# sjz5202/DisenLink

Measured on NVIDIA B200. Metric: factor-agg edges/s (fwd+bwd), higher is better.
Workload: dtype f32

## Files before the change

### disenlink_b200/csrc/attn_sym.cu

```cuda
#include "dl_dispatch.cuh"
#include "dl_prims.cuh"
#include "dl_stream.cuh"

namespace {

inline int blocks_for(long long n, int threads = 256) {
  long long b = (n + threads - 1) / threads;
  if (b < 1) b = 1;
  if (b > 148 * 32) b = 148 * 32;
  return (int)b;
}

__device__ __forceinline__ bool dl_primary(const long long* __restrict__ rowptr, int i, int j) {
  if (i == j) return true;
  const long long di = __ldg(rowptr + i + 1) - __ldg(rowptr + i), dj = __ldg(rowptr + j + 1) - __ldg(rowptr + j);
  return di > dj || (di == dj && i < j);
}

struct PrimaryFlag {
  const long long* rowptr;
  const int* col;
  const int* erow;
  long long nnz;
  __device__ __forceinline__ int operator()(long long e) const {
    return (e < nnz && dl_primary(rowptr, erow[e], col[e])) ? 1 : 0;
  }
};

__global__ void k_sym_uptr(const long long* __restrict__ rowptr, const int* __restrict__ pos, long long N,
                           long long* __restrict__ uptr) {
  const long long stride = (long long)gridDim.x * blockDim.x;
  for (long long r = (long long)blockIdx.x * blockDim.x + threadIdx.x; r <= N; r += stride) uptr[r] = pos[rowptr[r]];
}

__global__ void k_sym_fill(const long long* __restrict__ rowptr, const int* __restrict__ col,
                           const int* __restrict__ erow, long long nnz, const int* __restrict__ pos,
                           int* __restrict__ ucol, int* __restrict__ eidx,
                           int* __restrict__ lcol, int* __restrict__ lmirror, int* __restrict__ status,
                           unsigned long long* __restrict__ n_diag) {
  const long long stride = (long long)gridDim.x * blockDim.x;
  for (long long e = (long long)blockIdx.x * blockDim.x + threadIdx.x; e < nnz; e += stride) {
    const int i = erow[e], j = col[e];
    if (j == i) atomicAdd(n_diag, 1ULL);
    const int t = pos[e];
    if (pos[e + 1] != t) {
      ucol[t] = j;
      eidx[e] = t;
    } else {
      long long a = rowptr[j], b = rowptr[j + 1];
      const long long b0 = b;
      while (a < b) {
        const long long mid = (a + b) >> 1;
        if (col[mid] < i) a = mid + 1; else b = mid;
      }
      int m = 0;
      if (a < b0 && col[a] == i && pos[a + 1] != pos[a]) {
        m = pos[a];
      } else {
        *status = DL_EASYM;
      }
      eidx[e] = ~m;
      if (lcol) {
        lcol[e - t] = j;
        lmirror[e - t] = m;
      }
    }
  }
}

__global__ void k_sym_check(long long nnz, const int* __restrict__ pos,
                            const unsigned long long* __restrict__ n_diag, int* __restrict__ status) {
  const long long nu = pos[nnz];
  if (nnz - nu != nu - (long long)*n_diag) *status = DL_EASYM;
}

constexpr int SX_WARPS = 8;

template <int KP>
__global__ void __launch_bounds__(SX_WARPS * 32)
k_sym_expand(DlGraphDev g, const int* __restrict__ eidx, const float2* __restrict__ kw, int K,
             unsigned char* __restrict__ kstar, float* __restrict__ w, float* __restrict__ s,
             float* __restrict__ carry) {
  const int lane = threadIdx.x & 31;
  const long long gw = (long long)blockIdx.x * SX_WARPS + (threadIdx.x >> 5);
  const long long RE = (long long)DL_CH * DL_RANGE;
  DlChunkStream cs;
  cs.init(g.nnz, (long long)gridDim.x * SX_WARPS, g.range_shift);

  constexpr int NG = 32 / KP;
  const int grp = lane / KP, kap = lane % KP;
  float acc = 0.0f;
  int cur_row = -1;
  bool first_run = true, head_open = false, tail_open = false;
  long long cur_range = -1;
  auto flush = [&](bool at_range_end) {
    if (cur_row >= 0) {
      float v = acc;
#pragma unroll
      for (int off = KP; off < 32; off <<= 1) v = __fadd_rn(v, __shfl_xor_sync(DL_FULL, v, off));
      const bool to_head = first_run && head_open;
      const bool to_tail = !to_head && at_range_end && tail_open;
      if (grp == 0 && kap < K) {
        if (to_head || to_tail) carry[(cur_range * 2 + (to_tail ? 1 : 0)) * K + kap] = v;
        else s[(g.row_base + cur_row) * K + kap] = (v == 0.0f) ? 1.0f : v;
      }
      first_run = false;
    }
    cur_row = -1;
    acc = 0.0f;
  };

  struct Meta { int row, idx; };
  auto load_meta = [&](long long cc, Meta& m) {
    m.row = -1; m.idx = 0;
    if (cc >= 0) {
      const long long e = cc * DL_CH + lane;
      if (e < g.nnz) {
        m.row = __ldg(g.erow + e);
        const int t = __ldg(eidx + e);
        m.idx = t < 0 ? ~t : t;
      }
    }
  };
  auto gather = [&](const Meta& m) {
    float2 v = make_float2(0.0f, 0.0f);
    if (m.row >= 0) {
      asm volatile("ld.global.nc.L2::64B.v2.f32 {%0,%1}, [%2];" : "=f"(v.x), "=f"(v.y) : "l"(kw + m.idx));
    }
    return v;
  };

  long long c = cs.first(gw);
  Meta mA, mB, mC;
  load_meta(c, mA);
  long long cn = cs.next(c);
  load_meta(cn, mB);
  float2 vA = gather(mA), vB;
  while (c >= 0) {
    const long long cnn = cs.next(cn);
    load_meta(cnn, mC);
    vB = gather(mB);
    const long long rg = c >> g.range_shift;
    if (rg != cur_range) {
      if (cur_range >= 0) flush(true);
      cur_range = rg;
      first_run = true;
      const long long R0 = rg * RE, R1 = min(R0 + RE, g.nnz);
      head_open = R0 > 0 && __ldg(g.erow + R0 - 1) == __ldg(g.erow + R0);
      tail_open = R1 < g.nnz && __ldg(g.erow + R1) == __ldg(g.erow + R1 - 1);
    }
    const int ks = __float_as_int(vA.y);
    if (mA.row >= 0) {
      const long long e = c * DL_CH + lane;
      kstar[e] = (unsigned char)ks;
      w[e] = vA.x;
    }
    const unsigned vmask = __ballot_sync(DL_FULL, mA.row >= 0);
    const int cnt = __popc(vmask);
    for (int q = 0; q < cnt; q += NG) {
      const int src = q + grp;
      const int row_e = __shfl_sync(DL_FULL, mA.row, src & 31);
      const int ks_e = __shfl_sync(DL_FULL, ks, src & 31);
      const float w_e = __shfl_sync(DL_FULL, vA.x, src & 31);
      const bool valid = src < cnt;
      const float contrib = (valid && kap == ks_e) ? w_e : 0.0f;
      if (!__any_sync(DL_FULL, valid && row_e != cur_row)) {
        acc = __fadd_rn(acc, contrib);
      } else {
#pragma unroll 1
        for (int t = 0; t < NG && q + t < cnt; ++t) {
          const int re = __shfl_sync(DL_FULL, mA.row, q + t);
          if (re != cur_row) { flush(false); cur_row = re; }
          if (grp == t) acc = __fadd_rn(acc, contrib);
        }
      }
    }
    c = cn; cn = cnn;
    mA = mB; mB = mC;
    vA = vB;
  }
  if (cur_range >= 0) flush(true);
}

}

extern "C" {

size_t dl_sym_index_workspace_bytes(int64_t N, int64_t nnz) {
  if (N < 0 || nnz < 0) return 0;
  return dlp::align256((size_t)(nnz + 2) * 4) + dlp::scan_ws_bytes(nnz + 1, 4) + 256;
}

int dl_sym_index(const int64_t* rowptr, const int32_t* col, const int32_t* erow, int64_t N, int64_t nnz,
                 int64_t* uptr, int32_t* ucol, int32_t* eidx, int32_t* lcol, int32_t* lmirror, int32_t* status_out,
                 void* ws, size_t ws_bytes, dl_stream_t stream) {
  if (N < 0 || nnz < 0 || !rowptr || !uptr || !ws || (nnz > 0 && (!col || !erow))) return DL_EINVAL;
  if (ws_bytes < dl_sym_index_workspace_bytes(N, nnz)) return DL_EWORKSPACE;
  if (nnz >= 0x7fffffffLL) return DL_EUNSUPPORTED;
  cudaStream_t st = (cudaStream_t)stream;
  int* pos = (int*)ws;
  void* scan_ws = (char*)ws + dlp::align256((size_t)(nnz + 2) * 4);
  int rc = dlp::scan<false, int>(PrimaryFlag{(const long long*)rowptr, col, erow, nnz}, dlp::StoreArr<int>{pos}, nnz + 1,
                                 dlp::OpSum<int>(), 0, scan_ws, st);
  if (rc) return rc;
  if (!ucol) {
    k_sym_uptr<<<blocks_for(N + 1), 256, 0, st>>>((const long long*)rowptr, pos, N, (long long*)uptr);
    DL_LAUNCH_CHECK();
    return DL_OK;
  }
  if (!eidx || !status_out || ((lcol == nullptr) != (lmirror == nullptr))) return DL_EINVAL;
  DL_CUDA_TRY(cudaMemsetAsync(status_out, 0, sizeof(int32_t), st));
  unsigned long long* n_diag =
      (unsigned long long*)((char*)ws + dlp::align256((size_t)(nnz + 2) * 4) + dlp::scan_ws_bytes(nnz + 1, 4));
  DL_CUDA_TRY(cudaMemsetAsync(n_diag, 0, sizeof(unsigned long long), st));
  if (nnz > 0) {
    k_sym_fill<<<blocks_for(nnz), 256, 0, st>>>((const long long*)rowptr, col, erow, nnz, pos, ucol, eidx, lcol,
                                                lmirror, status_out, n_diag);
    DL_LAUNCH_CHECK();
    k_sym_check<<<1, 1, 0, st>>>(nnz, pos, n_diag, status_out);
    DL_LAUNCH_CHECK();
  }
  return DL_OK;
}

int dl_edge_attn_fwd_sym(const dl_graph* g_host, const dl_graph* upper_host, const int32_t* eidx, const float* Z,
                         int K, int d, float T, uint8_t* kstar, float* w, float* s, float* hub_ws, float* kw_scratch,
                         float* a_out, dl_stream_t stream) {
  if (!dl_graph_ok(g_host) || !dl_graph_ok(upper_host) || !dl_shape_ok(K, d)) return DL_EINVAL;
  if (g_host->N == 0) return DL_OK;
  if (g_host->row_base != 0 || upper_host->row_base != 0 || upper_host->N != g_host->N) return DL_EINVAL;
  if (!Z || !s || (g_host->nnz > 0 && (!kstar || !w || !eidx || !kw_scratch || !hub_ws))) return DL_EINVAL;
  if (!g_host->erow || !upper_host->erow) return DL_EINVAL;
  if (!(T == T) || T == 0.0f) return DL_EINVAL;
  if (!dl_attn_fl_has(K, d) || g_host->nnz == 0) return DL_EUNSUPPORTED;
  cudaStream_t st = (cudaStream_t)stream;
  const DlGraphDev g = dl_graph_dev(g_host);
  const DlGraphDev gu = dl_graph_dev(upper_host);
  float2* kw = reinterpret_cast<float2*>(kw_scratch);
  if (g_host->flags & DL_F_NO_KEEPA) a_out = nullptr;
  int rc = dl_launch_attn_fl(gu, Z, K, d, T, nullptr, nullptr, nullptr, nullptr, st, kw, a_out);
  if (rc == -1000) return DL_EUNSUPPORTED;
  if (rc) return rc;
  int dev = 0, sms = 0;
  DL_CUDA_TRY(cudaGetDevice(&dev));
  DL_CUDA_TRY(cudaDeviceGetAttribute(&sms, cudaDevAttrMultiProcessorCount, dev));
  const long long n_chunks = (g.nnz + DL_CH - 1) / DL_CH;
  const long long n_ranges = (n_chunks + DL_RANGE - 1) / DL_RANGE;
  long long grid = (n_ranges + SX_WARPS - 1) / SX_WARPS;
  if (grid > (long long)sms * 8) grid = (long long)sms * 8;
  if (grid < 1) grid = 1;
  if (K <= 8) k_sym_expand<8><<<(int)grid, SX_WARPS * 32, 0, st>>>(g, eidx, kw, K, kstar, w, s, hub_ws);
  else k_sym_expand<32><<<(int)grid, SX_WARPS * 32, 0, st>>>(g, eidx, kw, K, kstar, w, s, hub_ws);
  DL_LAUNCH_CHECK();
  return dl_gather_chain_rowsum(g, K, hub_ws, s, st);
}

}
```

### disenlink_b200/csrc/factor_fwd.cu

```cuda
#include <math_constants.h>
#include <stdlib.h>

#include "dl_dispatch.cuh"

namespace {

template <class M>
__global__ void __launch_bounds__(DL_CTA_S)
k_edge_attn_fwd(DlGraphDev g, const float* __restrict__ Z, float T, unsigned char* __restrict__ kstar,
                float* __restrict__ w, float* __restrict__ s, float* __restrict__ hub_ws) {
  constexpr int K = M::K, D = M::D, NP = M::NP, EB = M::EB, LP = M::LP, FPP = M::FPP;
  const int lane = threadIdx.x & 31;
  const long long warp0 = (long long)blockIdx.x * DL_WARPS_PER_CTA_S + (threadIdx.x >> 5);
  const long long nwarps = (long long)gridDim.x * DL_WARPS_PER_CTA_S;

  int off[NP];
  bool act[NP];
#pragma unroll
  for (int p = 0; p < NP; ++p) { off[p] = M::offset(lane, p); act[p] = M::active(lane, p); }
  const int my_e = M::edge_of_lane(lane);
  const int gsrc = lane & (EB - 1);
  const bool primary = (lane % LP) < EB;
  const bool unit_T = (T == 1.0f);

  auto fetch = [&](float4 (&dst)[EB][NP], int colreg, int idx0, int lim) {
#pragma unroll
    for (int e = 0; e < EB; ++e) {
      const int idx = idx0 + e;
      const int c = __shfl_sync(DL_FULL, colreg, idx & 31);
      const bool valid = idx < lim;
#pragma unroll
      for (int p = 0; p < NP; ++p)
        dst[e][p] = (valid && act[p]) ? dl_ldg4(Z + (long long)c * D + off[p]) : dl_zero4();
    }
  };

  DlRowIter itr;
  itr.init(g, warp0, nwarps);
  DlItem it, nit;
  it = nit = DlItem{0, 0, 0, 0, -1};
  bool have = itr.next(g, it);
  int colA = 0;
  if (have && lane < it.e1 - it.e0) colA = __ldg(g.col + it.e0 + lane);
  float4 zjA[EB][NP], zjB[EB][NP];
  bool pre = false;

  while (have) {
    const bool have_n = itr.next(g, nit);
    const int ncntB = have_n ? (int)min(32LL, nit.e1 - nit.e0) : 0;
    int colB = 0;
    if (lane < ncntB) colB = __ldg(g.col + nit.e0 + lane);
    float4 zi[NP];
#pragma unroll
    for (int p = 0; p < NP; ++p) zi[p] = act[p] ? dl_ldg4(Z + it.node * D + off[p]) : dl_zero4();
    if (!pre && it.e1 > it.e0) fetch(zjA, colA, 0, (int)min(32LL, it.e1 - it.e0));
    bool pre_n = false;

    float sacc[NP];
#pragma unroll
    for (int p = 0; p < NP; ++p) sacc[p] = 0.0f;
    int mycol = colA, colN = 0;
    for (long long base = it.e0; base < it.e1; base += 32) {
      const int cnt = (int)min(32LL, it.e1 - base);
      const bool more = base + 32 < it.e1;
      const int ncntN = more ? (int)min(32LL, it.e1 - base - 32) : 0;
      if (lane < ncntN) colN = __ldg(g.col + base + 32 + lane);
      int out_ks = 0;
      float out_w = 0.0f;
      const int nsub = (cnt + EB - 1) / EB;
      for (int sb = 0; sb < nsub; ++sb) {
        {
          int pc, pi0, plim;
          if (sb + 1 < nsub) { pc = mycol; pi0 = (sb + 1) * EB; plim = cnt; }
          else if (more) { pc = colN; pi0 = 0; plim = ncntN; }
          else { pc = colB; pi0 = 0; plim = ncntB; pre_n = ncntB > 0; }
          fetch(zjB, pc, pi0, plim);
        }
        float ev[NP];
#pragma unroll
        for (int p = 0; p < NP; ++p) {
          float part[EB];
#pragma unroll
          for (int e = 0; e < EB; ++e) part[e] = dl_chunk_dot(zi[p], zjA[e][p]);
          float q = dl_reduce_scatter<M>(part, lane);
          if (!unit_T) q = __fdiv_rn(q, T);
          ev[p] = dl_expf(q);
        }
        float a[K];
        float sum = 0.0f;
#pragma unroll
        for (int k = 0; k < K; ++k) {
          a[k] = __shfl_sync(DL_FULL, ev[k / FPP], (k % FPP) * LP + gsrc);
          sum = (k == 0) ? a[0] : __fadd_rn(sum, a[k]);
        }
        int ks = 0;
        float emax = a[0];
#pragma unroll
        for (int k = 1; k < K; ++k)
          if (a[k] > emax) { emax = a[k]; ks = k; }
        const float thr = __fmul_rn(emax, 0.99999976158142089844f);
        bool slow = !(sum < CUDART_INF_F);
#pragma unroll
        for (int k = 0; k < K; ++k) slow = slow || (a[k] > thr && a[k] != emax);
        float wv;
        if (!slow) {
          wv = __fdiv_rn(emax, sum);
        } else {
          ks = 0;
          wv = 0.0f;
#pragma unroll
          for (int k = 0; k < K; ++k) {
            float v = __fdiv_rn(a[k], sum);
            if (k == 0) { wv = v; }
            else if (v > wv || (v != v && wv == wv)) { wv = v; ks = k; }
          }
        }
        const bool valid = (sb * EB + my_e) < cnt;
#pragma unroll
        for (int p = 0; p < NP; ++p)
          if (valid && primary && ks == M::factor(lane, p)) sacc[p] = __fadd_rn(sacc[p], wv);
        if (sb == lane / EB) { out_ks = ks; out_w = wv; }
#pragma unroll
        for (int e = 0; e < EB; ++e)
#pragma unroll
          for (int p = 0; p < NP; ++p) zjA[e][p] = zjB[e][p];
      }
      const int oi = (lane & ~(EB - 1)) + my_e;
      if (oi < cnt) {
        kstar[base + oi] = (unsigned char)out_ks;
        w[base + oi] = out_w;
      }
      mycol = colN;
    }
#pragma unroll
    for (int p = 0; p < NP; ++p) {
      float v = sacc[p];
#pragma unroll
      for (int o = 1; o < EB; o <<= 1) v = __fadd_rn(v, __shfl_xor_sync(DL_FULL, v, o));
      const int k = M::factor(lane, p);
      if (k < K && (lane % LP) == 0) {
        if (it.hub_slot >= 0) hub_ws[it.hub_slot * K + k] = v;
        else s[it.node * K + k] = (v == 0.0f) ? 1.0f : v;
      }
    }
    it = nit;
    have = have_n;
    colA = colB;
    pre = pre_n;
  }
}

__global__ void __launch_bounds__(DL_CTA)
k_edge_attn_fwd_generic(DlGraphDev g, const float* __restrict__ Z, int K, int d, float T,
                        unsigned char* __restrict__ kstar, float* __restrict__ w,
                        float* __restrict__ s, float* __restrict__ hub_ws) {
  const int lane = threadIdx.x & 31;
  const long long warp0 = (long long)blockIdx.x * DL_WARPS_PER_CTA + (threadIdx.x >> 5);
  const long long nwarps = (long long)gridDim.x * DL_WARPS_PER_CTA;
  const long long n_items = dl_num_items(g);
  const long long D = (long long)K * d;
  float e[DL_MAX_K], a[DL_MAX_K], sacc[DL_MAX_K];
  for (long long t = warp0; t < n_items; t += nwarps) {
    const DlItem it = dl_decode_item(g, t);
    for (int k = 0; k < K; ++k) sacc[k] = 0.0f;
    const float* zi = Z + it.node * D;
    for (long long p = it.e0; p < it.e1; ++p) {
      const float* zj = Z + (long long)__ldg(g.col + p) * D;
      int ks = dl_generic_route(zi, zj, K, d, T, lane, e, a);
      float wv = a[ks];
      sacc[ks] = __fadd_rn(sacc[ks], wv);
      if (lane == 0) { kstar[p] = (unsigned char)ks; w[p] = wv; }
    }
    if (lane == 0) {
      for (int k = 0; k < K; ++k) {
        if (it.hub_slot >= 0) hub_ws[it.hub_slot * K + k] = sacc[k];
        else s[it.node * K + k] = (sacc[k] == 0.0f) ? 1.0f : sacc[k];
      }
    }
  }
}

__global__ void k_attn_hub_fixup(DlGraphDev g, int K, const float* __restrict__ hub_ws,
                                 float* __restrict__ s) {
  long long stride = (long long)gridDim.x * blockDim.x;
  for (long long x = (long long)blockIdx.x * blockDim.x + threadIdx.x; x < g.n_hub * K; x += stride) {
    long long h = x / K;
    int k = (int)(x % K);
    long long a = g.hub_seg_ptr[h], b = g.hub_seg_ptr[h + 1];
    float v = 0.0f;
    for (long long sg = a; sg < b; ++sg) v = __fadd_rn(v, hub_ws[sg * K + k]);
    s[(g.row_base + g.perm[h]) * K + k] = (v == 0.0f) ? 1.0f : v;
  }
}

__global__ void __launch_bounds__(DL_CTA)
k_factor_spmm_fwd_generic(DlGraphDev g, const float* __restrict__ Z,
                          const unsigned char* __restrict__ kstar, const float* __restrict__ w,
                          const float* __restrict__ s, int K, int d, float beta, float omb,
                          float* __restrict__ H, float* __restrict__ hub_ws) {
  const int lane = threadIdx.x & 31;
  const long long warp0 = (long long)blockIdx.x * DL_WARPS_PER_CTA + (threadIdx.x >> 5);
  const long long nwarps = (long long)gridDim.x * DL_WARPS_PER_CTA;
  const long long n_items = dl_num_items(g);
  const long long D = (long long)K * d;
  for (long long t = warp0; t < n_items; t += nwarps) {
    const DlItem it = dl_decode_item(g, t);
    float* acc = it.hub_slot >= 0 ? hub_ws + it.hub_slot * D : H + it.node * D;
    for (long long x = lane; x < D; x += 32) acc[x] = 0.0f;
    __syncwarp();
    for (long long p = it.e0; p < it.e1; ++p) {
      const long long j = __ldg(g.col + p);
      const int k = __ldg(kstar + p);
      const float coef = __fdiv_rn(__ldg(w + p), __ldg(s + j * K + k));
      const float* zj = Z + j * D + (long long)k * d;
      float* ak = acc + (long long)k * d;
      for (int x = lane; x < d; x += 32) ak[x] = __fmaf_rn(coef, zj[x], ak[x]);
    }
    __syncwarp();
    if (it.hub_slot < 0) {
      const float* zi = Z + it.node * D;
      for (long long x = lane; x < D; x += 32)
        acc[x] = __fadd_rn(__fmul_rn(beta, zi[x]), __fmul_rn(omb, acc[x]));
    }
  }
}

__global__ void k_spmm_hub_fixup(DlGraphDev g, long long D, const float* __restrict__ Z,
                                 const float* __restrict__ hub_ws, float beta, float omb,
                                 float* __restrict__ H) {
  long long stride = (long long)gridDim.x * blockDim.x;
  for (long long x = (long long)blockIdx.x * blockDim.x + threadIdx.x; x < g.n_hub * D; x += stride) {
    long long h = x / D, o = x % D;
    long long a = g.hub_seg_ptr[h], b = g.hub_seg_ptr[h + 1];
    float v = 0.0f;
    for (long long sg = a; sg < b; ++sg) v = __fadd_rn(v, hub_ws[sg * D + o]);
    long long row = g.row_base + g.perm[h];
    H[row * D + o] = __fadd_rn(__fmul_rn(beta, Z[row * D + o]), __fmul_rn(omb, v));
  }
}

template <class M>
int launch_attn(const DlGraphDev& g, long long n_items, const float* Z, float T, uint8_t* kstar,
                float* w, float* s, float* hub_ws, cudaStream_t st) {
  int grid = 1;
  int rc = dl_grid_for(k_edge_attn_fwd<M>, n_items, &grid, 0, DL_CTA_S);
  if (rc) return rc;
  k_edge_attn_fwd<M><<<grid, DL_CTA_S, 0, st>>>(g, Z, T, kstar, w, s, hub_ws);
  DL_LAUNCH_CHECK();
  return DL_OK;
}

inline int fixup_blocks(long long n) {
  long long b = (n + 255) / 256;
  if (b < 1) b = 1;
  if (b > 148 * 16) b = 148 * 16;
  return (int)b;
}

}

static __global__ void __launch_bounds__(256)
k_scale_rows(const float* __restrict__ Z, const float* __restrict__ s, long long n_rows, int K, int d,
             float* __restrict__ Zs) {
  const int lane = threadIdx.x & 31;
  const int D4 = K * d / 4, d4 = d / 4;
  const long long nwarps = (long long)gridDim.x * (blockDim.x >> 5);
  for (long long row = (long long)blockIdx.x * (blockDim.x >> 5) + (threadIdx.x >> 5); row < n_rows; row += nwarps) {
    const float4* zr = reinterpret_cast<const float4*>(Z) + row * D4;
    float4* out = reinterpret_cast<float4*>(Zs) + row * D4;
    for (int c = lane; c < D4; c += 32) {
      const float rs = __fdiv_rn(1.0f, __ldg(s + row * K + c / d4));
      float4 v = __ldg(zr + c);
      v.x = __fmul_rn(v.x, rs); v.y = __fmul_rn(v.y, rs); v.z = __fmul_rn(v.z, rs); v.w = __fmul_rn(v.w, rs);
      out[c] = v;
    }
  }
}

static __global__ void k_entry_sj(DlGraphDev g, const unsigned char* __restrict__ kstar, const float* __restrict__ s,
                           int K, float* __restrict__ sj) {
  const long long stride = (long long)gridDim.x * blockDim.x;
  for (long long e = (long long)blockIdx.x * blockDim.x + threadIdx.x; e < g.nnz; e += stride)
    sj[e] = __ldg(s + (long long)__ldg(g.col + e) * K + __ldg(kstar + e));
}

extern "C" {

size_t dl_hub_scratch_floats(const dl_graph* g_host, int64_t width) {
  if (!g_host || width < 0) return 0;
  const size_t hub = (size_t)g_host->n_hub_items * (size_t)width;
  const long long RE = 32LL << dl_range_shift(g_host->nnz);
  const size_t stream = (size_t)((g_host->nnz + RE - 1) / RE) * 3 * (size_t)width;
  return hub > stream ? hub : stream;
}

static int attn_fwd_impl(const dl_graph* g_host, const float* Z, int K, int d, float T,
                         uint8_t* kstar, float* w, float* s, float* hub_ws, float* const* s_peers, int n_peers,
                         dl_stream_t stream) {
  if (!dl_graph_ok(g_host) || !dl_shape_ok(K, d)) return DL_EINVAL;
  if (g_host->N == 0) return DL_OK;
  if (!Z || !s || (g_host->nnz > 0 && (!kstar || !w))) return DL_EINVAL;
  if (g_host->n_hub_items > 0 && !hub_ws) return DL_EINVAL;
  if (!(T == T) || T == 0.0f) return DL_EINVAL;
  cudaStream_t st = (cudaStream_t)stream;
  const unsigned flags = g_host->flags;
  const bool no_stream = (flags & DL_F_NO_STREAM) != 0;
  DlGraphDev g = dl_graph_dev(g_host);
  if (!dl_set_peer_out(g, s_peers, n_peers)) return DL_EINVAL;
  const long long n_items = g.n_hub_items + (g.N - g.n_hub);
  int rc = -1000;
  bool stream_tried = false;
  if (g.erow && g.nnz > 0 && !(flags & (DL_F_NO_STREAM | DL_F_NO_FL | DL_F_NO_FL_ATTN))) {
    rc = dl_launch_attn_fl(g, Z, K, d, T, kstar, w, s, hub_ws, st);
    if (rc == DL_OK) return DL_OK;
    if (rc != -1000) return rc;
  }
  if (g.erow && g.nnz > 0 && !no_stream) {
    rc = dl_launch_attn_stream(g, g.erow, Z, K, d, T, kstar, w, s, hub_ws, st);
    stream_tried = (rc != -1000);
  }
  if (rc == -1000) {
#define BODY_MACRO(M) rc = launch_attn<M>(g, n_items, Z, T, kstar, w, s, hub_ws, st);
    DL_DISPATCH_SHAPES()
#undef BODY_MACRO
  }
  if (rc == -1000) {
    int grid = 1;
    rc = dl_grid_for(k_edge_attn_fwd_generic, n_items, &grid);
    if (rc) return rc;
    k_edge_attn_fwd_generic<<<grid, DL_CTA, 0, st>>>(g, Z, K, d, T, kstar, w, s, hub_ws);
    DL_LAUNCH_CHECK();
    rc = DL_OK;
  }
  bool streamed = false;
  if (rc == -1001) { rc = DL_OK; }
  else if (rc == DL_OK && g.erow && g.nnz > 0 && !no_stream && stream_tried) streamed = true;
  if (rc) return rc;
  if (g.n_hub > 0 && !streamed) {
    k_attn_hub_fixup<<<fixup_blocks(g.n_hub * K), 256, 0, st>>>(g, K, hub_ws, s);
    DL_LAUNCH_CHECK();
  }
  if (n_peers > 0 && !streamed) {
    void* dst[DL_MAX_PEER_OUT];
    const long long off = g.row_base * (long long)K;
    for (int q = 0; q < n_peers; ++q) dst[q] = s_peers[q] + off;
    return dl_push_slice(s + off, dst, n_peers, (int64_t)g.N * K * 4, stream);
  }
  return DL_OK;
}

int dl_edge_attn_fwd(const dl_graph* g_host, const float* Z, int K, int d, float T,
                     uint8_t* kstar, float* w, float* s, float* hub_ws, dl_stream_t stream) {
  return attn_fwd_impl(g_host, Z, K, d, T, kstar, w, s, hub_ws, nullptr, 0, stream);
}

int dl_edge_attn_fwd_push(const dl_graph* g_host, const float* Z, int K, int d, float T,
                          uint8_t* kstar, float* w, float* s, float* hub_ws, float* const* s_peers, int n_peers,
                          dl_stream_t stream) {
  return attn_fwd_impl(g_host, Z, K, d, T, kstar, w, s, hub_ws, s_peers, n_peers, stream);
}

static int spmm_fwd_impl(const dl_graph* g_host, const float* Z, const uint8_t* kstar,
                         const float* w, const float* s, int K, int d, float beta,
                         float one_minus_beta, float* H, float* sj_out, float* zs_scratch, int64_t zs_rows,
                         float* hub_ws, float* const* H_peers, int n_peers, dl_stream_t stream) {
  if (!dl_graph_ok(g_host) || !dl_shape_ok(K, d)) return DL_EINVAL;
  if (g_host->N == 0) return DL_OK;
  if (!Z || !s || !H || (g_host->nnz > 0 && (!kstar || !w))) return DL_EINVAL;
  if (g_host->n_hub_items > 0 && !hub_ws) return DL_EINVAL;
  cudaStream_t st = (cudaStream_t)stream;
  const unsigned flags = g_host->flags;
  DlGraphDev g = dl_graph_dev(g_host);
  if (!dl_set_peer_out(g, H_peers, n_peers)) return DL_EINVAL;
  const long long n_items = g.n_hub_items + (g.N - g.n_hub);
  int rc = -1000;
  if (zs_scratch && (sj_out || g.row_base != 0)) return DL_EINVAL;
  if (zs_scratch && g.nnz > 0 && d % 4 == 0 && g.erow && !(flags & (DL_F_NO_STREAM | DL_F_NO_PRESCALE))) {
    k_scale_rows<<<148 * 16, 256, 0, st>>>(Z, s, zs_rows > g.N ? zs_rows : g.N, K, d, zs_scratch);
    DL_LAUNCH_CHECK();
    rc = dl_launch_gather_stream(0, g, Z, zs_scratch, kstar, w, nullptr, K, d, beta, one_minus_beta, H, nullptr,
                                 hub_ws, st);
    if (rc == DL_OK) return DL_OK;
    if (rc != -1000) return rc;
  }
  if (!(flags & DL_F_NO_STREAM))
    rc = dl_launch_gather_stream(0, g, Z, Z, kstar, w, s, K, d, beta, one_minus_beta, H, sj_out, hub_ws, st);
  if (rc == DL_OK) return DL_OK;
  if (rc != -1000) return rc;
  if (sj_out && g.nnz > 0) {
    k_entry_sj<<<fixup_blocks(g.nnz), 256, 0, st>>>(g, kstar, s, K, sj_out);
    DL_LAUNCH_CHECK();
  }
  rc = dl_launch_slice_gather(0, g, n_items, Z, Z, kstar, w, s, K, d, beta, one_minus_beta, H, nullptr,
                              hub_ws, st);
  if (rc == -1000) {
    int grid = 1;
    rc = dl_grid_for(k_factor_spmm_fwd_generic, n_items, &grid);
    if (rc) return rc;
    k_factor_spmm_fwd_generic<<<grid, DL_CTA, 0, st>>>(g, Z, kstar, w, s, K, d, beta, one_minus_beta,
                                                       H, hub_ws);
    DL_LAUNCH_CHECK();
    rc = DL_OK;
  }
  if (rc) return rc;
  if (g.n_hub > 0) {
    const long long D = (long long)K * d;
    k_spmm_hub_fixup<<<fixup_blocks(g.n_hub * D), 256, 0, st>>>(g, D, Z, hub_ws, beta, one_minus_beta, H);
    DL_LAUNCH_CHECK();
  }
  if (n_peers > 0) {
    void* dst[DL_MAX_PEER_OUT];
    const long long off = g.row_base * (long long)K * d;
    for (int q = 0; q < n_peers; ++q) dst[q] = H_peers[q] + off;
    return dl_push_slice(H + off, dst, n_peers, (int64_t)g.N * K * d * 4, stream);
  }
  return DL_OK;
}

int dl_factor_spmm_fwd(const dl_graph* g_host, const float* Z, const uint8_t* kstar,
                       const float* w, const float* s, int K, int d, float beta,
                       float one_minus_beta, float* H, float* sj_out, float* zs_scratch, int64_t zs_rows,
                       float* hub_ws, dl_stream_t stream) {
  return spmm_fwd_impl(g_host, Z, kstar, w, s, K, d, beta, one_minus_beta, H, sj_out, zs_scratch, zs_rows, hub_ws,
                       nullptr, 0, stream);
}

int dl_factor_spmm_fwd_push(const dl_graph* g_host, const float* Z, const uint8_t* kstar,
                            const float* w, const float* s, int K, int d, float beta,
                            float one_minus_beta, float* H, float* sj_out, float* hub_ws,
                            float* const* H_peers, int n_peers, dl_stream_t stream) {
  return spmm_fwd_impl(g_host, Z, kstar, w, s, K, d, beta, one_minus_beta, H, sj_out, nullptr, 0, hub_ws, H_peers,
                       n_peers, stream);
}

}
```

### disenlink_b200/csrc/gather_stream.cu

```cuda
#ifndef DL_CPA_L2
#define DL_CPA_L2 ".L2::64B"
#endif
#ifndef DL_LDG_L2
#define DL_LDG_L2 ".L2::64B"
#endif
#include "dl_dispatch.cuh"
#include "dl_stream.cuh"
#include "dl_fl.cuh"

namespace {

constexpr int GS_WARPS = 16;

__device__ __forceinline__ float gs_ldg_s(const float* p) {
  float v;
  asm volatile("ld.global.nc" DL_LDG_L2 ".f32 %0, [%1];" : "=f"(v) : "l"(p));
  return v;
}

__host__ __device__ constexpr int carry_width(int mode, int K, int d) {
  return mode == 2 ? K : (mode == 4 ? 2 * K * d : K * d);
}

__device__ __forceinline__ void epilogue_flat(const DlGraphDev& g, int mode, int lane, long long node, int K, int d,
                                              const float* acc ,
                                              const float* __restrict__ Z, const float* __restrict__ G,
                                              const float* __restrict__ s, float beta, float omb,
                                              float* __restrict__ OUT, float* __restrict__ r) {
  const long long D = (long long)K * d;
  if (mode == 4) {
    for (long long x = lane; x < D; x += 32) {
      const float dh = acc ? acc[D + x] : 0.0f;
      OUT[node * D + x] = acc ? acc[x] : 0.0f;
      r[node * D + x] = dh;
      for (int q = 0; q < g.n_peer_out; ++q) g.peer_out[q][node * D + x] = dh;
    }
  } else if (mode == 3) {
    if (acc)
      for (long long x = lane; x < D; x += 32) OUT[node * D + x] = __fadd_rn(OUT[node * D + x], acc[x]);
  } else if (mode == 2) {
    for (int k = lane; k < K; k += 32) {
      const float v = acc ? acc[k] : 0.0f;
      const float sv = (v == 0.0f) ? 1.0f : v;
      OUT[node * K + k] = sv;
      for (int q = 0; q < g.n_peer_out; ++q) g.peer_out[q][node * K + k] = sv;
    }
  } else if (mode == 0) {
    for (long long x = lane; x < D; x += 32) {
      const float v = acc ? acc[x] : 0.0f;
      const float h = __fadd_rn(__fmul_rn(beta, Z[node * D + x]), __fmul_rn(omb, v));
      OUT[node * D + x] = h;
      for (int q = 0; q < g.n_peer_out; ++q) g.peer_out[q][node * D + x] = h;
    }
  } else {
    for (int k = 0; k < K; ++k) {
      const float sk = s[node * K + k];
      const float scale = __fdiv_rn(omb, sk);
      float part = 0.0f;
      for (int x = lane; x < d; x += 32) {
        const long long o = node * D + (long long)k * d + x;
        const float tv = __fmul_rn(scale, acc ? acc[(long long)k * d + x] : 0.0f);
        part = __fmaf_rn(Z[o], tv, part);
        OUT[o] = __fadd_rn(OUT[o], __fmaf_rn(beta, G[o], tv));
      }
      for (int o = 16; o > 0; o >>= 1) part = __fadd_rn(part, __shfl_xor_sync(DL_FULL, part, o));
      if (lane == 0) {
        const float rv = __fdiv_rn(part, sk);
        r[node * K + k] = rv;
        for (int q = 0; q < g.n_peer_out; ++q) g.peer_out[q][node * K + k] = rv;
      }
    }
  }
}

__global__ void __launch_bounds__(DL_CTA)
k_gather_empty_rows(DlGraphDev g, int mode, int K, int d, const float* __restrict__ Z,
                    const float* __restrict__ G, const float* __restrict__ s, float beta, float omb,
                    float* __restrict__ OUT, float* __restrict__ r) {
  const int lane = threadIdx.x & 31;
  const long long warp0 = (long long)blockIdx.x * DL_WARPS_PER_CTA + (threadIdx.x >> 5);
  const long long nwarps = (long long)gridDim.x * DL_WARPS_PER_CTA;
  for (long long r0 = warp0 * 32; r0 < g.N; r0 += nwarps * 32) {
    const long long row = r0 + lane;
    const bool empty = row < g.N && __ldg(g.rowptr + row) == __ldg(g.rowptr + row + 1);
    unsigned m = __ballot_sync(DL_FULL, empty);
    while (m) {
      const int l = __ffs(m) - 1;
      m &= m - 1;
      epilogue_flat(g, mode, lane, g.row_base + r0 + l, K, d, nullptr, Z, G, s, beta, omb, OUT, r);
    }
  }
}

__global__ void __launch_bounds__(DL_CTA)
k_gather_chain(DlGraphDev g, int mode, int K, int d, const float* __restrict__ carry,
               const float* __restrict__ Z, const float* __restrict__ G, const float* __restrict__ s,
               float beta, float omb, float* __restrict__ OUT, float* __restrict__ r,
               float* __restrict__ scratch ) {
  const int lane = threadIdx.x & 31;
  const long long warp0 = (long long)blockIdx.x * DL_WARPS_PER_CTA + (threadIdx.x >> 5);
  const long long nwarps = (long long)gridDim.x * DL_WARPS_PER_CTA;
  const int W = carry_width(mode, K, d);
  const long long RE = (long long)DL_CH * DL_RANGE;
  const long long n_ranges = (g.nnz + RE - 1) / RE;
  for (long long b = warp0; b < n_ranges; b += nwarps) {
    const long long R1 = min((b + 1) * RE, g.nnz);
    if (R1 >= g.nnz) continue;
    const int row = __ldg(g.erow + R1 - 1);
    if (__ldg(g.erow + R1) != row) continue;
    if (__ldg(g.rowptr + row) < b * RE) continue;
    const long long last = (__ldg(g.rowptr + row + 1) - 1) / RE;
    float* acc = scratch + b * W;
    for (int x0 = 0; x0 < W; x0 += 256) {
      float v[8];
#pragma unroll
      for (int j = 0; j < 8; ++j) {
        const int x = x0 + j * 32 + lane;
        v[j] = x < W ? carry[(b * 2 + 1) * W + x] : 0.0f;
      }
      long long bb = b + 1;
      for (; bb + 3 <= last; bb += 4) {
        float t[4][8];
#pragma unroll
        for (int u = 0; u < 4; ++u)
#pragma unroll
          for (int j = 0; j < 8; ++j) {
            const int x = x0 + j * 32 + lane;
            t[u][j] = x < W ? carry[((bb + u) * 2) * W + x] : 0.0f;
          }
#pragma unroll
        for (int u = 0; u < 4; ++u)
#pragma unroll
          for (int j = 0; j < 8; ++j) v[j] = __fadd_rn(v[j], t[u][j]);
      }
      for (; bb <= last; ++bb)
#pragma unroll
        for (int j = 0; j < 8; ++j) {
          const int x = x0 + j * 32 + lane;
          if (x < W) v[j] = __fadd_rn(v[j], carry[(bb * 2) * W + x]);
        }
#pragma unroll
      for (int j = 0; j < 8; ++j) {
        const int x = x0 + j * 32 + lane;
        if (x < W) acc[x] = v[j];
      }
    }
    __syncwarp();
    epilogue_flat(g, mode, lane, g.row_base + row, K, d, acc, Z, G, s, beta, omb, OUT, r);
  }
}

template <class M, int MODE>
struct GatherStreamCfg {
  static constexpr int SLB = M::d * 4;
  static constexpr int TILE_B = (MODE == 2) ? 0 : DL_CH * SLB;
  static constexpr int CF_B = (MODE == 2) ? 0 : DL_CH * 4;
  static constexpr int X_B = (MODE == 1) ? DL_CH * 4 : 0;
  static constexpr int WARP_B = 2 * TILE_B + CF_B + X_B;
  static constexpr size_t SMEM = (size_t)GS_WARPS * WARP_B;
};

template <class M, int MODE>
__global__ void __launch_bounds__(GS_WARPS * 32, (M::NP == 1) ? 2 : 1)
k_gather_stream(DlGraphDev g, const float* __restrict__ Z, const float* __restrict__ SRC,
                const unsigned char* __restrict__ kstar, const float* __restrict__ w,
                const float* __restrict__ s, float beta, float omb, float* __restrict__ OUT,
                float* __restrict__ r, float* __restrict__ carry, float* __restrict__ xout,
                const int* __restrict__ xidx, unsigned char* __restrict__ ku_out) {
  using C = GatherStreamCfg<M, MODE>;
  constexpr int K = M::K, d = M::d, D = M::D, NP = M::NP, L = M::L, LP = M::LP, FPP = M::FPP;
  constexpr int NG = 32 / LP, SLB = C::SLB, TILE_B = C::TILE_B;
  constexpr int W = (MODE == 2) ? K : D;
  extern __shared__ __align__(128) unsigned char dl_smem_raw[];
  const int lane = threadIdx.x & 31, warp = threadIdx.x >> 5;
  unsigned char* tile = dl_smem_raw + (size_t)warp * C::WARP_B;
  float* cfbuf = reinterpret_cast<float*>(tile + 2 * TILE_B);
  float* xbuf = cfbuf + DL_CH;
  const long long gw = (long long)blockIdx.x * GS_WARPS + warp;
  const int grp = lane / LP, gg = lane % LP, slot = M::slot(lane);
  const bool glane = gg < L;
  const long long RE = (long long)DL_CH * DL_RANGE;
  const unsigned gmask = (LP >= 32) ? 0xffffffffu : (((1u << LP) - 1u) << (grp * LP));
  const bool want_x = (MODE == 1) && (L == LP) && xout != nullptr;

  DlChunkStream cs;
  cs.init(g.nnz, (long long)gridDim.x * GS_WARPS, g.range_shift);

  struct Meta { int row, col, ks; float wv; };
  auto load_meta = [&](long long cc, Meta& m) {
    m.row = -1; m.col = 0; m.ks = 255; m.wv = 0.0f;
    if (cc >= 0) {
      const long long e = cc * DL_CH + lane;
      if (e < g.nnz) {
        m.row = __ldg(g.erow + e);
        m.ks = __ldg(kstar + e);
        m.wv = __ldg(w + e);
        if (MODE != 2) m.col = __ldg(g.col + e);
      }
    }
  };
  auto issue_slices = [&](unsigned char* buf, const Meta& m) {
    if (MODE == 2) return;
#pragma unroll
    for (int rd = 0; rd < LP; ++rd) {
      const int idx = rd * NG + grp;
      const int cc = __shfl_sync(DL_FULL, m.col, idx);
      const int kk = __shfl_sync(DL_FULL, m.ks, idx);
      if (glane && kk < K)
        dl_cp_async16(buf + idx * SLB + gg * 16, SRC + (long long)cc * D + kk * d + gg * 4);
    }
  };

  float4 acc[NP];
  float acc2 = 0.0f;
#pragma unroll
  for (int p = 0; p < NP; ++p) acc[p] = dl_zero4();
  int cur_row = -1;
  float4 zpre[NP], gpre[NP];
  float skpre[NP];
#pragma unroll
  for (int p = 0; p < NP; ++p) { zpre[p] = gpre[p] = dl_zero4(); skpre[p] = 1.0f; }
  auto prefetch_row = [&](int row) {
    if (MODE == 2) return;
    const long long node = g.row_base + row;
#pragma unroll
    for (int p = 0; p < NP; ++p) {
      if (!M::active(lane, p)) continue;
      const int o = M::offset(lane, p);
      zpre[p] = dl_ldg4(Z + node * D + o);
      if (MODE == 1) gpre[p] = dl_ldg4(SRC + node * D + o);
    }
    if (MODE == 1) {
#pragma unroll
      for (int p = 0; p < NP; ++p) {
        const int k = M::factor(lane, p);
        skpre[p] = (k < K) ? __ldg(s + node * K + k) : 1.0f;
      }
    }
  };
  bool first_run = true;
  bool head_open = false, tail_open = false;
  long long cur_range = -1;

  auto flush = [&](bool at_range_end) {
    if (cur_row >= 0) {
      const bool to_head = first_run && head_open;
      const bool to_tail = !to_head && at_range_end && tail_open;
      if (to_head || to_tail) {
        float* dst = carry + (cur_range * 2 + (to_tail ? 1 : 0)) * W;
        if (MODE == 2) {
          if (lane < K) dst[lane] = acc2;
        } else {
#pragma unroll
          for (int p = 0; p < NP; ++p)
            if (M::active(lane, p)) *reinterpret_cast<float4*>(dst + M::offset(lane, p)) = acc[p];
        }
      } else {
        const long long node = g.row_base + cur_row;
        if (MODE == 2) {
          if (lane < K) {
            const float sv = (acc2 == 0.0f) ? 1.0f : acc2;
            OUT[node * K + lane] = sv;
            for (int q = 0; q < g.n_peer_out; ++q) g.peer_out[q][node * K + lane] = sv;
          }
        } else if (MODE == 0) {
#pragma unroll
          for (int p = 0; p < NP; ++p) {
            if (!M::active(lane, p)) continue;
            const int o = M::offset(lane, p);
            const float4 zi = zpre[p];
            float4 h;
            h.x = __fadd_rn(__fmul_rn(beta, zi.x), __fmul_rn(omb, acc[p].x));
            h.y = __fadd_rn(__fmul_rn(beta, zi.y), __fmul_rn(omb, acc[p].y));
            h.z = __fadd_rn(__fmul_rn(beta, zi.z), __fmul_rn(omb, acc[p].z));
            h.w = __fadd_rn(__fmul_rn(beta, zi.w), __fmul_rn(omb, acc[p].w));
            *reinterpret_cast<float4*>(OUT + node * D + o) = h;
#pragma unroll 1
            for (int q = 0; q < g.n_peer_out; ++q)
              *reinterpret_cast<float4*>(g.peer_out[q] + node * D + o) = h;
          }
        } else {
#pragma unroll
          for (int p = 0; p < NP; ++p) {
            const int k = M::factor(lane, p);
            const bool act = M::active(lane, p);
            const int o = M::offset(lane, p);
            const float sk = skpre[p];
            const float scale = __fdiv_rn(omb, sk);
            float4 tv;
            tv.x = __fmul_rn(scale, acc[p].x); tv.y = __fmul_rn(scale, acc[p].y);
            tv.z = __fmul_rn(scale, acc[p].z); tv.w = __fmul_rn(scale, acc[p].w);
            const float4 zi = act ? zpre[p] : dl_zero4();
            const float dotzt = dl_group_sum<M>(dl_chunk_dot(zi, tv));
            if (k < K && gg == 0) {
              const float rv = __fdiv_rn(dotzt, sk);
              r[node * K + k] = rv;
              for (int q = 0; q < g.n_peer_out; ++q) g.peer_out[q][node * K + k] = rv;
            }
            if (act) {
              const float4 gi = gpre[p];
              float4 add;
              add.x = __fmaf_rn(beta, gi.x, tv.x); add.y = __fmaf_rn(beta, gi.y, tv.y);
              add.z = __fmaf_rn(beta, gi.z, tv.z); add.w = __fmaf_rn(beta, gi.w, tv.w);
              fl_red_add4(OUT + node * D + o, add);
            }
          }
        }
      }
    }
    if (cur_row >= 0) first_run = false;
    cur_row = -1;
    acc2 = 0.0f;
#pragma unroll
    for (int p = 0; p < NP; ++p) acc[p] = dl_zero4();
  };

  long long c = cs.first(gw);
  Meta mA, mB, mC;
  load_meta(c, mA);
  long long cn = cs.next(c);
  load_meta(cn, mB);
  float sjA = 1.0f, sjB = 1.0f;
  if (MODE == 0 && s != nullptr && mA.ks != 255) sjA = gs_ldg_s(s + (long long)mA.col * K + mA.ks);
  int buf = 0;
  issue_slices(tile, mA);
  dl_cp_async_commit();

  while (c >= 0) {
    const long long cnn = cs.next(cn);
    load_meta(cnn, mC);
    if (MODE == 0 && s != nullptr && mB.ks != 255) sjB = gs_ldg_s(s + (long long)mB.col * K + mB.ks);
    issue_slices(tile + (buf ^ 1) * TILE_B, mB);
    dl_cp_async_commit();
    dl_cp_async_wait<1>();
    __syncwarp();

    const long long rg = c >> g.range_shift;
    if (rg != cur_range) {
      if (cur_range >= 0) flush(true);
      cur_range = rg;
      first_run = true;
      const long long R0 = rg * RE, R1 = min(R0 + RE, g.nnz);
      head_open = R0 > 0 && __ldg(g.erow + R0 - 1) == __ldg(g.erow + R0);
      tail_open = R1 < g.nnz && __ldg(g.erow + R1) == __ldg(g.erow + R1 - 1);
    }

    if (MODE == 0 && r != nullptr && s != nullptr && mA.row >= 0) r[c * DL_CH + lane] = sjA;
    const float coefA = (MODE == 0) ? __fdiv_rn(mA.wv, sjA) : mA.wv;
    const unsigned vmask = __ballot_sync(DL_FULL, mA.row >= 0);
    const int cnt = __popc(vmask);
    const unsigned char* sl = tile + buf * TILE_B;
    const int prow = __shfl_up_sync(DL_FULL, mA.row, 1);
    const bool st = mA.row >= 0 && (lane == 0 ? mA.row != cur_row : mA.row != prow);
    const unsigned starts = __ballot_sync(DL_FULL, st);
    int idx = 0;
    if (MODE == 2) {
      while (idx < cnt) {
        if ((starts >> idx) & 1u) {
          flush(false);
          cur_row = __shfl_sync(DL_FULL, mA.row, idx);
        }
        const unsigned rest = (idx < 31) ? (starts & ~((2u << idx) - 1u)) : 0u;
        const int end = rest ? (__ffs(rest) - 1) : cnt;
        for (; idx < end; ++idx) {
          const unsigned ke = (unsigned)__shfl_sync(DL_FULL, mA.ks, idx);
          const float cf = __shfl_sync(DL_FULL, coefA, idx);
          if ((unsigned)lane == ke) acc2 = __fadd_rn(acc2, cf);
        }
      }
    } else {
      cfbuf[lane] = coefA;
      unsigned mine[NP];
#pragma unroll
      for (int p = 0; p < NP; ++p) mine[p] = 0u;
#pragma unroll
      for (int k = 0; k < K; ++k) {
        const unsigned b = __ballot_sync(DL_FULL, mA.ks == k);
        if (glane && slot == (k % FPP)) mine[k / FPP] = b;
      }
      __syncwarp();
      while (idx < cnt) {
        if ((starts >> idx) & 1u) {
          flush(false);
          cur_row = __shfl_sync(DL_FULL, mA.row, idx);
          prefetch_row(cur_row);
        }
        const unsigned rest = (idx < 31) ? (starts & ~((2u << idx) - 1u)) : 0u;
        const int end = rest ? (__ffs(rest) - 1) : cnt;
        const unsigned runbits = ((end < 32) ? ((1u << end) - 1u) : 0xffffffffu) & ~((1u << idx) - 1u);
#pragma unroll
        for (int p = 0; p < NP; ++p) {
          unsigned m = mine[p] & runbits;
          while (m) {
            const int i = __ffs(m) - 1;
            m &= m - 1;
            const float cf = cfbuf[i];
            const float4 v = dl_lds4(sl + i * SLB + gg * 16);
            dl_fma4(acc[p], cf, v);
            if (MODE == 1 && want_x) {
              float pd = dl_chunk_dot(v, zpre[p]);
#pragma unroll
              for (int off = 1; off < LP; off <<= 1) pd = __fadd_rn(pd, __shfl_xor_sync(gmask, pd, off));
              if (gg == 0) xbuf[i] = pd;
            }
          }
        }
        idx = end;
      }
    }
    __syncwarp();
    if (MODE == 1 && want_x && mA.row >= 0) {
      if (xidx == nullptr) {
        xout[c * DL_CH + lane] = xbuf[lane];
      } else {
        const int t = __ldg(xidx + c * DL_CH + lane);
        if (t >= 0) {
          xout[t] = xbuf[lane];
          if (ku_out) ku_out[t] = (unsigned char)mA.ks;
        }
      }
    }
    buf ^= 1;
    c = cn; cn = cnn;
    mA = mB; mB = mC;
    sjA = sjB;
  }
  if (cur_range >= 0) flush(true);
  dl_cp_async_wait<0>();
}

template <class M, int MODE>
int launch_gather_stream(const DlGraphDev& g, const float* Z, const float* SRC,
                         const unsigned char* kstar, const float* w, const float* s, float beta,
                         float omb, float* OUT, float* r, float* carry, float* xout, const int* xidx,
                         unsigned char* ku_out, cudaStream_t st) {
  using C = GatherStreamCfg<M, MODE>;
  if (C::SMEM > 200 * 1024) return -1000;
  if (C::SMEM > 48 * 1024)
    DL_CUDA_TRY(cudaFuncSetAttribute(k_gather_stream<M, MODE>, cudaFuncAttributeMaxDynamicSharedMemorySize,
                                     (int)C::SMEM));
  int dev = 0, sms = 0, per_sm = 0;
  DL_CUDA_TRY(cudaGetDevice(&dev));
  DL_CUDA_TRY(cudaDeviceGetAttribute(&sms, cudaDevAttrMultiProcessorCount, dev));
  DL_CUDA_TRY(cudaOccupancyMaxActiveBlocksPerMultiprocessor(&per_sm, k_gather_stream<M, MODE>, GS_WARPS * 32,
                                                            C::SMEM));
  if (per_sm < 1) per_sm = 1;
  const long long n_chunks = (g.nnz + DL_CH - 1) / DL_CH;
  const long long n_ranges = (n_chunks + DL_RANGE - 1) / DL_RANGE;
  long long grid = (n_ranges + GS_WARPS - 1) / GS_WARPS;
  const long long cap = (long long)sms * per_sm;
  if (grid > cap) grid = cap;
  if (grid < 1) grid = 1;
  k_gather_stream<M, MODE><<<(int)grid, GS_WARPS * 32, C::SMEM, st>>>(g, Z, SRC, kstar, w, s, beta, omb, OUT,
                                                                     r, carry, xout, xidx, ku_out);
  DL_LAUNCH_CHECK();
  return DL_OK;
}

inline int small_grid(long long n_warps_wanted) {
  long long b = (n_warps_wanted + DL_WARPS_PER_CTA - 1) / DL_WARPS_PER_CTA;
  if (b < 1) b = 1;
  if (b > 148 * 8) b = 148 * 8;
  return (int)b;
}

}

size_t dl_gather_stream_scratch_floats(long long nnz, int mode, int K, int d) {
  const long long RE = (long long)DL_CH << dl_range_shift(nnz);
  const long long n_ranges = (nnz + RE - 1) / RE;
  return (size_t)n_ranges * 3 * (size_t)carry_width(mode, K, d);
}

int dl_launch_gather_stream(int mode, const DlGraphDev& g, const float* Z, const float* SRC,
                            const unsigned char* kstar, const float* w, const float* s, int K, int d,
                            float beta, float omb, float* OUT, float* r, float* scratch,
                            cudaStream_t st, float* xout, const int* xidx, unsigned char* ku_out) {
  if (!g.erow || g.nnz == 0 || !scratch) return -1000;
  const long long RE = (long long)DL_CH * DL_RANGE;
  const long long n_ranges = (g.nnz + RE - 1) / RE;
  const int W = carry_width(mode, K, d);
  float* carry = scratch;
  float* chain = scratch + (size_t)n_ranges * 2 * W;
  int rc = -1000;
#define BODY_MACRO(M)                                                                                       \
  rc = (mode == 0)   ? launch_gather_stream<M, 0>(g, Z, SRC, kstar, w, s, beta, omb, OUT, r, carry, nullptr, nullptr, nullptr, st)  \
       : (mode == 1) ? launch_gather_stream<M, 1>(g, Z, SRC, kstar, w, s, beta, omb, OUT, r, carry, xout, xidx, ku_out, st)     \
                     : launch_gather_stream<M, 2>(g, Z, SRC, kstar, w, s, beta, omb, OUT, r, carry, nullptr, nullptr, nullptr, st);
  DL_DISPATCH_SHAPES()
#undef BODY_MACRO
  if (rc != DL_OK) return rc;
  float* r_node = (mode == 0) ? nullptr : r;
  k_gather_chain<<<small_grid(n_ranges), DL_CTA, 0, st>>>(g, mode, K, d, carry, Z, SRC, s, beta, omb, OUT,
                                                          r_node, chain);
  DL_LAUNCH_CHECK();
  k_gather_empty_rows<<<small_grid((g.N + 31) / 32), DL_CTA, 0, st>>>(g, mode, K, d, Z, SRC, s, beta, omb,
                                                                     OUT, r_node);
  DL_LAUNCH_CHECK();
  return DL_OK;
}

bool dl_gather_stream_has_x(int K, int d) {
  bool has = false;
#define BODY_MACRO(M) has = (M::L == M::LP);
  DL_DISPATCH_SHAPES()
#undef BODY_MACRO
  return has;
}

int dl_gather_chain_add(const DlGraphDev& g, int K, int d, float* scratch, float* OUT, cudaStream_t st) {
  const long long RE = (long long)DL_CH * DL_RANGE;
  const long long n_ranges = (g.nnz + RE - 1) / RE;
  const int W = K * d;
  k_gather_chain<<<small_grid(n_ranges), DL_CTA, 0, st>>>(g, 3, K, d, scratch, nullptr, nullptr, nullptr, 0.0f,
                                                          0.0f, OUT, nullptr, scratch + (size_t)n_ranges * 2 * W);
  DL_LAUNCH_CHECK();
  return DL_OK;
}

int dl_gather_chain_pair(const DlGraphDev& g, int K, int d, float* scratch, float* dZ, float* dH,
                         cudaStream_t st) {
  const long long RE = (long long)DL_CH * DL_RANGE;
  const long long n_ranges = (g.nnz + RE - 1) / RE;
  const int W = 2 * K * d;
  k_gather_chain<<<small_grid(n_ranges), DL_CTA, 0, st>>>(g, 4, K, d, scratch, nullptr, nullptr, nullptr, 0.0f,
                                                          0.0f, dZ, dH, scratch + (size_t)n_ranges * 2 * W);
  DL_LAUNCH_CHECK();
  k_gather_empty_rows<<<small_grid((g.N + 31) / 32), DL_CTA, 0, st>>>(g, 4, K, d, nullptr, nullptr, nullptr,
                                                                     0.0f, 0.0f, dZ, dH);
  DL_LAUNCH_CHECK();
  return DL_OK;
}

int dl_gather_chain_rowsum(const DlGraphDev& g, int K, float* scratch, float* s_out, cudaStream_t st) {
  const long long RE = (long long)DL_CH * DL_RANGE;
  const long long n_ranges = (g.nnz + RE - 1) / RE;
  k_gather_chain<<<small_grid(n_ranges), DL_CTA, 0, st>>>(g, 2, K, 1, scratch, nullptr, nullptr, nullptr, 0.0f,
                                                          0.0f, s_out, nullptr, scratch + (size_t)n_ranges * 2 * K);
  DL_LAUNCH_CHECK();
  k_gather_empty_rows<<<small_grid((g.N + 31) / 32), DL_CTA, 0, st>>>(g, 2, K, 1, nullptr, nullptr, nullptr,
                                                                     0.0f, 0.0f, s_out, nullptr);
  DL_LAUNCH_CHECK();
  return DL_OK;
}
```

Baseline: 3.517 billion.

## Deepen gather prefetch pipelines and unroll scale/empty-row kernels

Extends the attention-symmetrize gather loop from a two-stage to a three-stage metadata/value prefetch, and gives the gather-stream cp.async ring a third buffer when d<=16, so more memory requests are in flight per warp. The row-scaling kernel is flattened to a grid-stride over float4 elements with 4-way unrolled loads and streaming cache hints. The empty-row scan now handles 128 rows per warp iteration with batched rowptr loads. In exchange it uses more registers and shared memory per warp, which may lower occupancy.

```diff
diff --git a/disenlink_b200/csrc/attn_sym.cu b/disenlink_b200/csrc/attn_sym.cu
--- a/disenlink_b200/csrc/attn_sym.cu
+++ b/disenlink_b200/csrc/attn_sym.cu
@@ -131,15 +131,17 @@
   };
 
   long long c = cs.first(gw);
-  Meta mA, mB, mC;
+  Meta mA, mB, mC, mD;
   load_meta(c, mA);
   long long cn = cs.next(c);
   load_meta(cn, mB);
-  float2 vA = gather(mA), vB;
+  long long cnn = cs.next(cn);
+  load_meta(cnn, mC);
+  float2 vA = gather(mA), vB = gather(mB), vC;
   while (c >= 0) {
-    const long long cnn = cs.next(cn);
-    load_meta(cnn, mC);
-    vB = gather(mB);
+    const long long c3 = cs.next(cnn);
+    load_meta(c3, mD);
+    vC = gather(mC);
     const long long rg = c >> g.range_shift;
     if (rg != cur_range) {
       if (cur_range >= 0) flush(true);
@@ -175,9 +177,9 @@
         }
       }
     }
-    c = cn; cn = cnn;
-    mA = mB; mB = mC;
-    vA = vB;
+    c = cn; cn = cnn; cnn = c3;
+    mA = mB; mB = mC; mC = mD;
+    vA = vB; vB = vC;
   }
   if (cur_range >= 0) flush(true);
 }
diff --git a/disenlink_b200/csrc/factor_fwd.cu b/disenlink_b200/csrc/factor_fwd.cu
--- a/disenlink_b200/csrc/factor_fwd.cu
+++ b/disenlink_b200/csrc/factor_fwd.cu
@@ -259,20 +259,36 @@
 
 }
 
+constexpr int SR_U = 4;
 static __global__ void __launch_bounds__(256)
 k_scale_rows(const float* __restrict__ Z, const float* __restrict__ s, long long n_rows, int K, int d,
              float* __restrict__ Zs) {
-  const int lane = threadIdx.x & 31;
   const int D4 = K * d / 4, d4 = d / 4;
-  const long long nwarps = (long long)gridDim.x * (blockDim.x >> 5);
-  for (long long row = (long long)blockIdx.x * (blockDim.x >> 5) + (threadIdx.x >> 5); row < n_rows; row += nwarps) {
-    const float4* zr = reinterpret_cast<const float4*>(Z) + row * D4;
-    float4* out = reinterpret_cast<float4*>(Zs) + row * D4;
-    for (int c = lane; c < D4; c += 32) {
-      const float rs = __fdiv_rn(1.0f, __ldg(s + row * K + c / d4));
-      float4 v = __ldg(zr + c);
-      v.x = __fmul_rn(v.x, rs); v.y = __fmul_rn(v.y, rs); v.z = __fmul_rn(v.z, rs); v.w = __fmul_rn(v.w, rs);
-      out[c] = v;
+  const long long n4 = n_rows * D4;
+  const long long stride = (long long)gridDim.x * blockDim.x;
+  const float4* zr = reinterpret_cast<const float4*>(Z);
+  float4* out = reinterpret_cast<float4*>(Zs);
+  for (long long i0 = (long long)blockIdx.x * blockDim.x + threadIdx.x; i0 < n4; i0 += SR_U * stride) {
+    float4 v[SR_U];
+    float sv[SR_U];
+#pragma unroll
+    for (int u = 0; u < SR_U; ++u) {
+      const long long i = i0 + u * stride;
+      if (i < n4) {
+        const long long row = i / D4;
+        sv[u] = __ldg(s + row * K + (int)(i - row * D4) / d4);
+        v[u] = __ldcs(zr + i);
+      }
+    }
+#pragma unroll
+    for (int u = 0; u < SR_U; ++u) {
+      const long long i = i0 + u * stride;
+      if (i < n4) {
+        const float rs = __fdiv_rn(1.0f, sv[u]);
+        float4 w = v[u];
+        w.x = __fmul_rn(w.x, rs); w.y = __fmul_rn(w.y, rs); w.z = __fmul_rn(w.z, rs); w.w = __fmul_rn(w.w, rs);
+        out[i] = w;
+      }
     }
   }
 }
diff --git a/disenlink_b200/csrc/gather_stream.cu b/disenlink_b200/csrc/gather_stream.cu
--- a/disenlink_b200/csrc/gather_stream.cu
+++ b/disenlink_b200/csrc/gather_stream.cu
@@ -80,14 +80,24 @@
   const int lane = threadIdx.x & 31;
   const long long warp0 = (long long)blockIdx.x * DL_WARPS_PER_CTA + (threadIdx.x >> 5);
   const long long nwarps = (long long)gridDim.x * DL_WARPS_PER_CTA;
-  for (long long r0 = warp0 * 32; r0 < g.N; r0 += nwarps * 32) {
-    const long long row = r0 + lane;
-    const bool empty = row < g.N && __ldg(g.rowptr + row) == __ldg(g.rowptr + row + 1);
-    unsigned m = __ballot_sync(DL_FULL, empty);
-    while (m) {
-      const int l = __ffs(m) - 1;
-      m &= m - 1;
-      epilogue_flat(g, mode, lane, g.row_base + r0 + l, K, d, nullptr, Z, G, s, beta, omb, OUT, r);
+  constexpr int U = 4;
+  for (long long r0 = warp0 * (32 * U); r0 < g.N; r0 += nwarps * (32 * U)) {
+    long long a[U], b[U];
+#pragma unroll
+    for (int u = 0; u < U; ++u) {
+      const long long row = min(r0 + u * 32 + lane, g.N - 1);
+      a[u] = __ldg(g.rowptr + row);
+      b[u] = __ldg(g.rowptr + row + 1);
+    }
+#pragma unroll
+    for (int u = 0; u < U; ++u) {
+      const long long rb = r0 + u * 32;
+      unsigned m = __ballot_sync(DL_FULL, rb + lane < g.N && a[u] == b[u]);
+      while (m) {
+        const int l = __ffs(m) - 1;
+        m &= m - 1;
+        epilogue_flat(g, mode, lane, g.row_base + rb + l, K, d, nullptr, Z, G, s, beta, omb, OUT, r);
+      }
     }
   }
 }
@@ -156,7 +166,8 @@
   static constexpr int TILE_B = (MODE == 2) ? 0 : DL_CH * SLB;
   static constexpr int CF_B = (MODE == 2) ? 0 : DL_CH * 4;
   static constexpr int X_B = (MODE == 1) ? DL_CH * 4 : 0;
-  static constexpr int WARP_B = 2 * TILE_B + CF_B + X_B;
+  static constexpr int RING = (M::d <= 16) ? 3 : 2;
+  static constexpr int WARP_B = RING * TILE_B + CF_B + X_B;
   static constexpr size_t SMEM = (size_t)GS_WARPS * WARP_B;
 };
 
@@ -174,7 +185,8 @@
   extern __shared__ __align__(128) unsigned char dl_smem_raw[];
   const int lane = threadIdx.x & 31, warp = threadIdx.x >> 5;
   unsigned char* tile = dl_smem_raw + (size_t)warp * C::WARP_B;
-  float* cfbuf = reinterpret_cast<float*>(tile + 2 * TILE_B);
+  constexpr int RING = C::RING;
+  float* cfbuf = reinterpret_cast<float*>(tile + RING * TILE_B);
   float* xbuf = cfbuf + DL_CH;
   const long long gw = (long long)blockIdx.x * GS_WARPS + warp;
   const int grp = lane / LP, gg = lane % LP, slot = M::slot(lane);
@@ -316,23 +328,42 @@
   };
 
   long long c = cs.first(gw);
-  Meta mA, mB, mC;
+  Meta mA, mB, mC, mD;
   load_meta(c, mA);
   long long cn = cs.next(c);
   load_meta(cn, mB);
-  float sjA = 1.0f, sjB = 1.0f;
+  long long cnn = -1, c3 = -1;
+  if (RING == 3) {
+    cnn = cs.next(cn);
+    load_meta(cnn, mC);
+  }
+  float sjA = 1.0f, sjB = 1.0f, sjC = 1.0f;
   if (MODE == 0 && s != nullptr && mA.ks != 255) sjA = gs_ldg_s(s + (long long)mA.col * K + mA.ks);
+  if (RING == 3 && MODE == 0 && s != nullptr && mB.ks != 255) sjB = gs_ldg_s(s + (long long)mB.col * K + mB.ks);
   int buf = 0;
   issue_slices(tile, mA);
   dl_cp_async_commit();
+  if (RING == 3) {
+    issue_slices(tile + TILE_B, mB);
+    dl_cp_async_commit();
+  }
 
   while (c >= 0) {
-    const long long cnn = cs.next(cn);
-    load_meta(cnn, mC);
-    if (MODE == 0 && s != nullptr && mB.ks != 255) sjB = gs_ldg_s(s + (long long)mB.col * K + mB.ks);
-    issue_slices(tile + (buf ^ 1) * TILE_B, mB);
-    dl_cp_async_commit();
-    dl_cp_async_wait<1>();
+    if (RING == 3) {
+      c3 = cs.next(cnn);
+      load_meta(c3, mD);
+      if (MODE == 0 && s != nullptr && mC.ks != 255) sjC = gs_ldg_s(s + (long long)mC.col * K + mC.ks);
+      issue_slices(tile + (buf == 0 ? 2 : buf - 1) * TILE_B, mC);
+      dl_cp_async_commit();
+      dl_cp_async_wait<2>();
+    } else {
+      cnn = cs.next(cn);
+      load_meta(cnn, mC);
+      if (MODE == 0 && s != nullptr && mB.ks != 255) sjB = gs_ldg_s(s + (long long)mB.col * K + mB.ks);
+      issue_slices(tile + (buf ^ 1) * TILE_B, mB);
+      dl_cp_async_commit();
+      dl_cp_async_wait<1>();
+    }
     __syncwarp();
 
     const long long rg = c >> g.range_shift;
@@ -420,10 +451,17 @@
         }
       }
     }
-    buf ^= 1;
-    c = cn; cn = cnn;
-    mA = mB; mB = mC;
-    sjA = sjB;
+    if (RING == 3) {
+      buf = (buf == 2) ? 0 : buf + 1;
+      c = cn; cn = cnn; cnn = c3;
+      mA = mB; mB = mC; mC = mD;
+      sjA = sjB; sjB = sjC;
+    } else {
+      buf ^= 1;
+      c = cn; cn = cnn;
+      mA = mB; mB = mC;
+      sjA = sjB;
+    }
   }
   if (cur_range >= 0) flush(true);
   dl_cp_async_wait<0>();
@@ -494,7 +532,7 @@
   k_gather_chain<<<small_grid(n_ranges), DL_CTA, 0, st>>>(g, mode, K, d, carry, Z, SRC, s, beta, omb, OUT,
                                                           r_node, chain);
   DL_LAUNCH_CHECK();
-  k_gather_empty_rows<<<small_grid((g.N + 31) / 32), DL_CTA, 0, st>>>(g, mode, K, d, Z, SRC, s, beta, omb,
+  k_gather_empty_rows<<<small_grid((g.N + 127) / 128), DL_CTA, 0, st>>>(g, mode, K, d, Z, SRC, s, beta, omb,
                                                                      OUT, r_node);
   DL_LAUNCH_CHECK();
   return DL_OK;
@@ -526,7 +564,7 @@
   k_gather_chain<<<small_grid(n_ranges), DL_CTA, 0, st>>>(g, 4, K, d, scratch, nullptr, nullptr, nullptr, 0.0f,
                                                           0.0f, dZ, dH, scratch + (size_t)n_ranges * 2 * W);
   DL_LAUNCH_CHECK();
-  k_gather_empty_rows<<<small_grid((g.N + 31) / 32), DL_CTA, 0, st>>>(g, 4, K, d, nullptr, nullptr, nullptr,
+  k_gather_empty_rows<<<small_grid((g.N + 127) / 128), DL_CTA, 0, st>>>(g, 4, K, d, nullptr, nullptr, nullptr,
                                                                      0.0f, 0.0f, dZ, dH);
   DL_LAUNCH_CHECK();
   return DL_OK;
@@ -538,7 +576,7 @@
   k_gather_chain<<<small_grid(n_ranges), DL_CTA, 0, st>>>(g, 2, K, 1, scratch, nullptr, nullptr, nullptr, 0.0f,
                                                           0.0f, s_out, nullptr, scratch + (size_t)n_ranges * 2 * K);
   DL_LAUNCH_CHECK();
-  k_gather_empty_rows<<<small_grid((g.N + 31) / 32), DL_CTA, 0, st>>>(g, 2, K, 1, nullptr, nullptr, nullptr,
+  k_gather_empty_rows<<<small_grid((g.N + 127) / 128), DL_CTA, 0, st>>>(g, 2, K, 1, nullptr, nullptr, nullptr,
                                                                      0.0f, 0.0f, s_out, nullptr);
   DL_LAUNCH_CHECK();
   return DL_OK;
```

Result: no change. 3.517 billion (median of 6 runs) (-0.0%).
